# gisbi-kim/lt-mapper

Measured on AMD Instinct MI355X. Metric: keyframe-pairs/sec (removert+diff), higher is better.
Workload: dtype f32; 1 GPU; lot-2x500-os1-64-3res; sensor=os1-64

## Files before the change

include/ltm.h:

```cpp
#ifndef LTM_H
#define LTM_H

#include <stddef.h>
#include <stdint.h>

#ifdef __cplusplus
extern "C" {
#endif

#define LTM_ABI_VERSION 1

enum {
    LTM_OK = 0,
    LTM_E_INVALID = -1,
    LTM_E_DEVICE = -2,
    LTM_E_NOMEM = -3,
    LTM_E_UNSUPPORTED = -4
};

typedef struct ltm_ctx ltm_ctx;
typedef uint64_t ltm_cloud;
typedef uint64_t ltm_scanset;
typedef uint64_t ltm_poses;

// ... 166 lines not shown
int ltm_debug_range_image(ltm_ctx*, ltm_cloud pts, const double* T1, const double* T2, float res_alpha,
                          float* rimg, int32_t* ptidx);
int ltm_debug_viz_images(ltm_ctx*, ltm_cloud map, ltm_scanset scans, ltm_poses poses, size_t kf, float res_alpha, int mode,
                         float range_min, float range_max, float diff_min, float diff_max,
                         uint8_t* scan_bgr, uint8_t* map_bgr, uint8_t* diff_bgr, uint8_t* ptidx_bgr);
int ltm_debug_project(ltm_ctx*, const float* xyz, size_t n, float res_alpha, float* out_az_el_r, int32_t* out_row_col);
void ltm_rimg_size(float vfov, float hfov, float res_alpha, int* rows, int* cols);
int ltm_debug_selfcheck(ltm_ctx*, uint64_t* mismatches3, int* fast_math_enabled);
int ltm_debug_elevation_fit(float vfov_deg, float* c4, double* max_err_rad);
int ltm_debug_pcl_sort_order(const uint32_t* leaf_idx, size_t n, uint32_t* order_out, int use_std_sort, uint32_t* heap_sort_fallbacks );
int ltm_debug_voxel_key_bits(const float* mn3, const float* mx3, float leaf, uint64_t* kept_mask, unsigned* depth, double* frame_min3);
int ltm_debug_cull_check(ltm_ctx*, const float* xyz, size_t n, const double* inv_pose16_or_null, float res_alpha, uint64_t* violations);
int ltm_debug_cull_validation(ltm_ctx*, uint64_t* shapes_checked, uint64_t* shapes_failed);
int ltm_debug_occlusion_stats(ltm_ctx*, uint64_t* pairs, uint64_t* first_shell, uint64_t* projected, int reset);
int ltm_debug_voxel_stats(ltm_ctx*, uint64_t* grids, uint64_t* identity_hits, int reset);
int ltm_debug_knn_stats(ltm_ctx*, uint64_t* queries, uint64_t* undecided, uint64_t* two_phase_calls, uint64_t* unsorted_queue_calls, int reset);
int ltm_debug_sc_paths(int num_ring, int num_sector, int* scatter_in_lds, int* pair_in_lds);
int ltm_debug_cull_stats(ltm_ctx*, uint64_t* survivors, uint64_t* points, int reset);
int ltm_debug_pool_live(ltm_ctx*, uint64_t* live_blocks, uint64_t* live_bytes);

int ltm_profile_enable(ltm_ctx*, int on);
int ltm_profile_reset(ltm_ctx*);
int ltm_profile_read(ltm_ctx*, const char** names, double* ms, uint64_t* launches, double* units, double* bytes, int cap);
int ltm_profile_read_compulsory(ltm_ctx*, double* bytes_c, int cap);

#ifdef __cplusplus
}
#endif
#endif
```

lt-mapper_amd/capi.py:

```python
import ctypes as C
import os

import numpy as np

_HERE = os.path.dirname(os.path.abspath(__file__))
LIB_PATH = os.path.join(_HERE, "libltm_hip.so")

_lib = None

LTM_OK = 0
ERR_NAMES = {0: "LTM_OK", -1: "LTM_E_INVALID", -2: "LTM_E_DEVICE", -3: "LTM_E_NOMEM", -4: "LTM_E_UNSUPPORTED"}


class LtmError(RuntimeError):
    def __init__(self, code, msg):
        super().__init__(f"{ERR_NAMES.get(code, code)}: {msg}")
        self.code = code


class LtmConfig(C.Structure):
    _fields_ = [("vfov", C.c_float), ("hfov", C.c_float), ("lidar2base", C.c_double * 16),
                ("device", C.c_int), ("max_kf_batch", C.c_int)]


# ... 116 lines not shown
    "ltm_submaps_assemble": (_i, [_vp, _u64, _vp, _vp, _sz, _i, _f, _i, _pu64]),
    "ltm_search_build_scanset": (_i, [_vp, _u64, _sz, _sz, C.POINTER(_vp)]),
    "ltm_debug_pool_live": (_i, [_vp, _pu64, _pu64]),
    "ltm_debug_range_image": (_i, [_vp, _u64, _vp, _vp, _f, _vp, _vp]),
    "ltm_debug_viz_images": (_i, [_vp, _u64, _u64, _u64, _sz, _f, _i, _f, _f, _f, _f, _vp, _vp, _vp, _vp]),
    "ltm_debug_project": (_i, [_vp, _vp, _sz, _f, _vp, _vp]),
    "ltm_debug_elevation_fit": (_i, [_f, C.POINTER(_f), C.POINTER(C.c_double)]),
    "ltm_debug_pcl_sort_order": (_i, [C.POINTER(C.c_uint32), C.c_size_t, C.POINTER(C.c_uint32), _i, C.POINTER(C.c_uint32)]),
    "ltm_debug_voxel_key_bits": (_i, [C.POINTER(_f), C.POINTER(_f), _f, _pu64, C.POINTER(C.c_uint), C.POINTER(C.c_double)]),
    "ltm_debug_selfcheck": (_i, [_vp, _pu64, C.POINTER(_i)]),
    "ltm_debug_cull_check": (_i, [_vp, _vp, _sz, _vp, _f, _pu64]),
    "ltm_debug_cull_stats": (_i, [_vp, _pu64, _pu64, _i]),
    "ltm_debug_cull_validation": (_i, [_vp, _pu64, _pu64]),
    "ltm_debug_occlusion_stats": (_i, [_vp, _pu64, _pu64, _pu64, _i]),
    "ltm_debug_voxel_stats": (_i, [_vp, _pu64, _pu64, _i]),
    "ltm_debug_knn_stats": (_i, [_vp, _pu64, _pu64, _pu64, _pu64, _i]),
    "ltm_debug_sc_paths": (_i, [_i, _i, C.POINTER(_i), C.POINTER(_i)]),
    "ltm_rimg_size": (None, [_f, _f, _f, C.POINTER(_i), C.POINTER(_i)]),
    "ltm_profile_enable": (_i, [_vp, _i]),
    "ltm_profile_reset": (_i, [_vp]),
    "ltm_profile_read_compulsory": (_i, [_vp, C.POINTER(C.c_double), _i]),
    "ltm_profile_read": (_i, [_vp, C.POINTER(C.c_char_p), C.POINTER(C.c_double), _pu64, C.POINTER(C.c_double),
                              C.POINTER(C.c_double), _i]),
}


def load_library(path=None):
    global _lib
    if _lib is not None and path is None:
        return _lib
# ... 460 lines not shown
        t = None if inv_pose is None else _mat16(inv_pose)
        v = _u64()
        self._ck(self.lib.ltm_debug_cull_check(self.h, a.ctypes.data, a.shape[0], None if t is None else t.ctypes.data, alpha, C.byref(v)))
        return int(v.value)

    def occlusion_stats(self, reset=False):
        a, b, d = _u64(), _u64(), _u64()
        self._ck(self.lib.ltm_debug_occlusion_stats(self.h, C.byref(a), C.byref(b), C.byref(d), 1 if reset else 0))
        return a.value, b.value, d.value

    def voxel_stats(self, reset=False):
        a, b = _u64(), _u64()
        self._ck(self.lib.ltm_debug_voxel_stats(self.h, C.byref(a), C.byref(b), 1 if reset else 0))
        return int(a.value), int(b.value)

    def knn_stats(self, reset=False):
        q, u, t, s = _u64(), _u64(), _u64(), _u64()
        self._ck(self.lib.ltm_debug_knn_stats(self.h, C.byref(q), C.byref(u), C.byref(t), C.byref(s), 1 if reset else 0))
        return int(q.value), int(u.value), int(t.value), int(s.value)

    def cull_validation(self):
        a, b = _u64(), _u64()
        self._ck(self.lib.ltm_debug_cull_validation(self.h, C.byref(a), C.byref(b)))
        return int(a.value), int(b.value)

    def cull_stats(self, reset=True):
        a, b = _u64(), _u64()
        self._ck(self.lib.ltm_debug_cull_stats(self.h, C.byref(a), C.byref(b), 1 if reset else 0))
        return int(a.value), int(b.value)

# ... 332 lines not shown
```

lt-mapper_amd/csrc/ltm_api_core.cpp:

```cpp
#include "ltm_internal.h"

namespace ltm_detail {

bool inverse4x4(const double* m, double* inv)
{
    double A[2][2], B[2][2], C[2][2], D[2][2];
    for (int r = 0; r < 2; ++r)
        for (int k = 0; k < 2; ++k) {
            A[r][k] = m[4 * k + r]; B[r][k] = m[4 * (k + 2) + r];
            C[r][k] = m[4 * k + r + 2]; D[r][k] = m[4 * (k + 2) + r + 2];
        }
    const double dA = A[0][0] * A[1][1] - A[0][1] * A[1][0], dB = B[0][0] * B[1][1] - B[0][1] * B[1][0];
    const double dC = C[0][0] * C[1][1] - C[0][1] * C[1][0], dD = D[0][0] * D[1][1] - D[0][1] * D[1][0];
    double AB[2][2], DC[2][2];
    for (int j = 0; j < 2; ++j) {
        AB[0][j] = B[0][j] * A[1][1] - B[1][j] * A[0][1]; AB[1][j] = B[1][j] * A[0][0] - B[0][j] * A[1][0];
        DC[0][j] = C[0][j] * D[1][1] - C[1][j] * D[0][1]; DC[1][j] = C[1][j] * D[0][0] - C[0][j] * D[1][0];
    }
    const double tr = (AB[0][0] * DC[0][0] + AB[1][0] * DC[0][1]) + (AB[0][1] * DC[1][0] + AB[1][1] * DC[1][1]);
    double iA[2][2], iB[2][2], iC[2][2], iD[2][2];
    for (int i = 0; i < 2; ++i)
        for (int j = 0; j < 2; ++j) {
            iD[i][j] = D[i][j] * dA - (AB[0][j] * C[i][0] + AB[1][j] * C[i][1]);
            iA[i][j] = A[i][j] * dD - (DC[0][j] * B[i][0] + DC[1][j] * B[i][1]);
// ... 193 lines not shown
    c->kopts.tile_cull = env_int("LTM_TILE_CULL", 1);
    c->kopts.stats_blockmin = env_int("LTM_STATS_BLOCKMIN", 0);
    {
        unsigned long long* d = nullptr;
        bool ok = hipMalloc(&d, 3 * sizeof(unsigned long long)) == hipSuccess && hipMemsetAsync(d, 0, 24, c->stream) == hipSuccess &&
                  selfcheck_fast_math(cfg->vfov, cfg->hfov, d, c->stream) == hipSuccess &&
                  hipMemcpyAsync(c->selfcheck, d, 24, hipMemcpyDeviceToHost, c->stream) == hipSuccess &&
                  hipStreamSynchronize(c->stream) == hipSuccess;
        if (d) (void)hipFree(d);
        if (!ok) { (void)hipStreamDestroy(c->stream); delete c; return LTM_E_DEVICE; }
        c->fast_math = (c->selfcheck[0] == 0 && c->selfcheck[1] == 0 && c->selfcheck[2] == 0) ? 1 : 0;
        if (const char* v = getenv("LTM_KNN_FAST")) c->knn_two_phase = atoi(v);
        if (const char* v = getenv("LTM_VOXEL_KEYBITS")) c->voxel_key_compress = atoi(v);
        if (const char* v = getenv("LTM_VOXEL_FUSED_TAIL")) c->voxel_fused_tail = atoi(v);
        if (const char* v = getenv("LTM_VOXEL_IDENTITY")) c->voxel_identity = atoi(v);
        if (const char* v = getenv("LTM_OCCLUSION")) c->occlusion_cull = atoi(v);
        if (getenv("LTM_OCCLUSION_STATS")) c->occlusion_stats_on = 1;
        if (const char* v = getenv("LTM_OCCLUSION_MIN_PAIRS")) c->occlusion_min_pairs = (size_t)atoll(v);
        if (const char* v = getenv("LTM_OCCLUSION_RNEAR")) {
            const float r = (float)atof(v);
            c->occlusion_r_near = std::isfinite(r) ? std::max(1.0f, r) : 60.0f;
        }
        if (const char* v = getenv("LTM_KNN_STATS")) c->knn_stats_on = atoi(v);
        if (const char* v = getenv("LTM_CULL_SELFCHECK")) c->cull_selfcheck = atoi(v);
        if (const char* v = getenv("LTM_CULL_EPS_SCALE")) c->cull_eps_scale = (float)atof(v);
        if (const char* v = getenv("LTM_CULL_EPS_FLOOR")) c->cull_eps_floor = (float)atof(v);
        c->el_fit = elevation_fit_for(c->cfg.vfov, c->el_c, &c->el_fit_err);
        if (const char* v = getenv("LTM_HEAVY_CHAIN")) c->heavy_chain_on = atoi(v);
        if (const char* v = getenv("LTM_HEAVY_MIN_BLOCKS")) c->heavy_min_blocks = (size_t)atoll(v);
    }
// ... 95 lines not shown
}

int ltm_cloud_device_ptr(ltm_ctx* c, ltm_cloud h, const void** p)
{
    return guarded(c, [&] { LTM_REQUIRE(p, "null argument"); *p = get_cloud(c, h).d; });
}

int ltm_cloud_clone(ltm_ctx* c, ltm_cloud h, ltm_cloud* out)
{
    return guarded(c, [&] {
        LTM_REQUIRE(out, "null argument");
        const Cloud src = get_cloud(c, h);
        float4* d;
        const ltm_cloud nh = alloc_cloud(c, src.n, &d);
        d2d(c, d, src.d, src.n * 16);
        inherit_frame(c, nh, src);
        *out = nh;
    });
}

int ltm_cloud_concat(ltm_ctx* c, const ltm_cloud* in, size_t n, ltm_cloud* out)
{
    return guarded(c, [&] {
        LTM_REQUIRE(out && (in || n == 0), "null argument");
        size_t tot = 0;
        for (size_t i = 0; i < n; ++i) tot += get_cloud(c, in[i]).n;
        float4* d;
        const ltm_cloud h = alloc_cloud(c, tot, &d);
        size_t at = 0;
        for (size_t i = 0; i < n; ++i) { const Cloud& s = get_cloud(c, in[i]); d2d(c, d + at, s.d, s.n * 16); at += s.n; }
        *out = h;
    });
}

int ltm_cloud_transform(ltm_ctx* c, ltm_cloud hin, const double* T1, const double* T2, ltm_cloud* out)
{
    return guarded(c, [&] {
        LTM_REQUIRE(out, "null argument");
        const Cloud in = get_cloud(c, hin);
        float4* d;
        const ltm_cloud h = alloc_cloud(c, in.n, &d);
        HostMat34 a, b;
        if (T1) a = to34(T1);
        if (T2) b = to34(T2);
        if (!T1 && !T2) d2d(c, d, in.d, in.n * 16);
// ... 572 lines not shown
{
    if (!parent || !out) return LTM_E_INVALID;
    *out = nullptr;
    ltm_ctx* c = new (std::nothrow) ltm_ctx();
    if (!c) return LTM_E_NOMEM;
    {
        std::lock_guard<std::recursive_mutex> lk(parent->mx);
        c->cfg = parent->cfg; c->device = parent->device; c->L2B = parent->L2B; c->B2L = parent->B2L;
        c->l2b_identity = parent->l2b_identity; c->b2l_identity = parent->b2l_identity; c->kf_batch = parent->kf_batch; c->kopts = parent->kopts;
        c->fast_math = parent->fast_math;
        for (int i = 0; i < 3; ++i) c->selfcheck[i] = parent->selfcheck[i];
        c->scan_cache_cap = parent->scan_cache_cap; c->occlusion_cull = parent->occlusion_cull;
        c->occlusion_min_pairs = parent->occlusion_min_pairs; c->occlusion_r_near = parent->occlusion_r_near;
        c->occlusion_subtile = parent->occlusion_subtile; c->occlusion_stats_on = parent->occlusion_stats_on;
        c->voxel_key_compress = parent->voxel_key_compress; c->voxel_fused_tail = parent->voxel_fused_tail; c->voxel_identity = parent->voxel_identity;
        c->knn_two_phase = parent->knn_two_phase; c->knn_stats_on = parent->knn_stats_on;
        c->cull_eps_scale = parent->cull_eps_scale; c->cull_eps_floor = parent->cull_eps_floor;
        c->cull_selfcheck = parent->cull_selfcheck; c->cull_geom_ok = parent->cull_geom_ok;
        c->el_fit = parent->el_fit; for (int i = 0; i < 4; ++i) c->el_c[i] = parent->el_c[i]; c->el_fit_err = parent->el_fit_err;
    }
    if (hipSetDevice(c->device) != hipSuccess || hipStreamCreateWithFlags(&c->stream, hipStreamNonBlocking) != hipSuccess) {
        delete c;
        return LTM_E_DEVICE;
    }
    c->pool.stream = c->stream;
    {
        std::lock_guard<std::recursive_mutex> lk(parent->mx);
        c->heavy = parent->heavy;
        c->heavy_chain_on = parent->heavy_chain_on; c->heavy_min_blocks = parent->heavy_min_blocks;
        c->in_lane_family = parent->in_lane_family = true;
// ... 32 lines not shown
    if (!ev) return;
    if (ev->e) { (void)hipSetDevice(ev->device); (void)hipEventDestroy(ev->e); }
    delete ev;
}

static int cloud_pass(ltm_ctx* from, ltm_cloud h, ltm_ctx* to, ltm_cloud* out, bool give)
{
    return guarded2(from, to, [&] {
        LTM_REQUIRE(out, "null argument");
        LTM_REQUIRE(from != to, "lend / give need two contexts");
        const Cloud src = get_cloud(from, h);
        LTM_REQUIRE(!give || !src.borrowed, "a borrowed cloud cannot be given away");
        stream_after(from, to);
        const ltm_cloud nh = new_cloud(to, src.d, src.n);
        Cloud& dst = to->clouds[nh];
        dst.vf_ok = src.vf_ok; dst.vf = src.vf; dst.vleaf = src.vleaf;
        if (give) {
            if (!from->pool.move_to(src.d, to->pool)) { to->clouds.erase(nh); throw Err{LTM_E_INVALID, "cloud memory is not owned by this context's pool"}; }
            from->clouds.erase(h);
        } else dst.borrowed = true;
        *out = nh;
    });
}

int ltm_cloud_lend(ltm_ctx* from, ltm_cloud h, ltm_ctx* to, ltm_cloud* out) { return cloud_pass(from, h, to, out, false); }

int ltm_cloud_give(ltm_ctx* from, ltm_cloud h, ltm_ctx* to, ltm_cloud* out) { return cloud_pass(from, h, to, out, true); }

static int scanset_pass(ltm_ctx* from, ltm_scanset h, ltm_ctx* to, ltm_scanset* out, bool give)
{
    return guarded2(from, to, [&] {
// ... 87 lines not shown
```

lt-mapper_amd/csrc/ltm_api_voxel.cpp:

```cpp
#include "ltm_internal.h"

namespace ltm_detail {

bool octree_frame_from_bbox(const float mn[3], const float mx[3], float leaf, OctreeFrame* f)
{
    const float eps512 = FLT_EPSILON * 512.0f;
    const float minValue = FLT_EPSILON;
    double lo[3], hi[3];
    for (int d = 0; d < 3; ++d) { lo[d] = (double)mn[d]; hi[d] = (double)(float)(mx[d] + eps512); }
    const double res = (double)leaf;
    unsigned mk = 2;
    for (int d = 0; d < 3; ++d) mk = std::max(mk, (unsigned)std::ceil((hi[d] - lo[d] - minValue) / res));
    const unsigned depth = std::min(32u, (unsigned)std::ceil(std::log2((double)mk) - minValue));
    if (depth > 21) return false;
    const double side = (double)(1u << depth) * res;
    for (int d = 0; d < 3; ++d) {
        const double over = (side - (hi[d] - lo[d])) / 2.0;
        if (over > minValue) lo[d] -= over;
    }
    f->minx = lo[0]; f->miny = lo[1]; f->minz = lo[2]; f->res = res; f->depth = depth;
    return true;
}

KeyCompress key_compress_for(const float mn[3], const float mx[3], const OctreeFrame& f, bool enable)
// ... 45 lines not shown
void voxel_segments(ltm_ctx* c, const uint64_t* keys2, size_t n, unsigned kshift, uint32_t* starts, uint32_t* count_dev)
{
    if (c->voxel_fused_tail) {
        const size_t tb = voxel_heads_starts_temp_bytes(n);
        DevBuf temp(c, tb);
        LTM_HIP(voxel_heads_starts(keys2, n, kshift, starts, temp.p, count_dev, c->stream));
        return;
    }
    DevBuf heads(c, n), pos(c, n * 4);
    LTM_HIP(head_flags(keys2, n, heads.as<uint8_t>(), c->stream, kshift));
    scan_flags(c, heads.as<uint8_t>(), n, pos);
    LTM_HIP(scan_total_to(heads.as<uint8_t>(), pos.as<uint32_t>(), n, count_dev, c->stream));
    LTM_HIP(segment_starts(heads.as<uint8_t>(), pos.as<uint32_t>(), n, starts, c->stream));
}

size_t voxel_centroid_raw(ltm_ctx* c, const float4* pts, size_t n_in, float leaf, float4** out, uint32_t shard = 0, uint32_t n_shards = 1,
                          const OctreeFrame* cached = nullptr, OctreeFrame* frame_out = nullptr, const float* box_mn = nullptr, const float* box_mx = nullptr)
{
    *out = nullptr;
    if (n_in == 0) return 0;
    LTM_REQUIRE(leaf > 0.0f, "leaf size must be positive");
    LTM_REQUIRE(n_in < 0xffffffffull, "cloud too large for 32-bit point indices");
    ProfScope p(c, "voxel", (double)n_in, 64.0 * n_in);
    ++c->voxel_calls;
    float mn[3], mx[3];
    bool untouched = false;
    if (cached && c->voxel_identity && n_shards == 1) {
        untouched = read_box(c, mn, mx, [&](uint32_t* bb) { return bbox_reduce_check(pts, n_in, *cached, bb, c->stream); }) == 0;
    } else if (box_mn && box_mx) {
        for (int d = 0; d < 3; ++d) { mn[d] = box_mn[d]; mx[d] = box_mx[d]; }
    } else bbox_of(c, pts, n_in, mn, mx);
    OctreeFrame f;
    if (!octree_frame_from_bbox(mn, mx, leaf, &f)) throw Err{LTM_E_UNSUPPORTED, "octree depth > 21 (extent / leaf too large)"};
    if (frame_out) *frame_out = f;
    if (untouched && same_frame(f, *cached)) {
        float4* o = reinterpret_cast<float4*>(c->pool.alloc(n_in * sizeof(float4)));
        d2d(c, o, pts, n_in * sizeof(float4));
        ++c->voxel_identity_hits;
        *out = o;
        return n_in;
    }
    unsigned ib = 1;
    while (ib < 32 && ((size_t)1 << ib) < n_in) ++ib;
    const KeyCompress kc = key_compress_for(mn, mx, f, c->voxel_key_compress != 0);
    const bool packed = kc.bits + ib <= 64;
    const unsigned mbits = packed ? kc.bits : 3 * f.depth;
    const unsigned kshift = packed ? ib : 0;
    size_t n = n_in;
    DevBuf keys(c, n * 8), idx(c, packed ? 8 : n * 4);
    if (packed) LTM_HIP(morton_keys_packed(pts, n, f, kc, ib, keys.as<uint64_t>(), c->stream));
    else LTM_HIP(morton_keys(pts, n, f, keys.as<uint64_t>(), idx.as<uint32_t>(), c->stream));
    if (n_shards > 1) {
        const unsigned shift = mbits > 12 ? mbits - 12 : 0;
        std::vector<uint32_t> hist(kVoxelKeyBins);
        {
            DevBuf hd(c, kVoxelKeyBins * sizeof(uint32_t));
            LTM_HIP(key_histogram(keys.as<uint64_t>(), n, shift + kshift, hd.as<uint32_t>(), c->stream));
            d2h(c, hist.data(), hd.p, kVoxelKeyBins * sizeof(uint32_t));
        }
        auto cut = [&](uint32_t b) -> uint64_t {
            if (b == 0) return 0;
            if (b >= n_shards) return kVoxelKeyBins;
// ... 8 lines not shown
        auto bound = [&](uint64_t bin) { return bin >= (uint64_t)kVoxelKeyBins ? ~0ull : bin << (shift + kshift); };
        const uint64_t lo = bound(cut(shard));
        const uint64_t hi = (shard + 1 >= n_shards) ? ~0ull : bound(cut(shard + 1));
        DevBuf flags(c, n), pos(c, n * 4);
        LTM_HIP(key_range_flags(keys.as<uint64_t>(), n, lo, hi, flags.as<uint8_t>(), c->stream));
        const size_t nsel = count_flags(c, flags.as<uint8_t>(), n, pos);
        if (nsel == 0) return 0;
        DevBuf ck(c, nsel * 8), ci(c, packed ? 8 : nsel * 4);
        if (packed) LTM_HIP(compact_keys(keys.as<uint64_t>(), flags.as<uint8_t>(), pos.as<uint32_t>(), n, ck.as<uint64_t>(), c->stream));
        else LTM_HIP(compact_pairs(keys.as<uint64_t>(), idx.as<uint32_t>(), flags.as<uint8_t>(), pos.as<uint32_t>(), n,
                                   ck.as<uint64_t>(), ci.as<uint32_t>(), c->stream));
        std::swap(keys.p, ck.p); std::swap(idx.p, ci.p);
        n = nsel;
    }
    DevBuf keys2(c, n * 8), idx2(c, packed ? 8 : n * 4);
    if (packed) {
        const size_t stb = sort_keys_temp_bytes(n);
        DevBuf stemp(c, stb);
        LTM_HIP(sort_keys_u64(keys.as<uint64_t>(), keys2.as<uint64_t>(), n, ib, ib + mbits, stemp.p, stb, c->stream));
    } else {
        const size_t stb = sort_temp_bytes(n);
        DevBuf stemp(c, stb);
        LTM_HIP(sort_pairs_u64(keys.as<uint64_t>(), keys2.as<uint64_t>(), idx.as<uint32_t>(), idx2.as<uint32_t>(), n, mbits, stemp.p, stb, c->stream));
    }
    DevBuf starts(c, n * 4), cnt(c, 4);
    voxel_segments(c, keys2.as<uint64_t>(), n, kshift, starts.as<uint32_t>(), cnt.as<uint32_t>());
    uint32_t nvox32 = 0;
    d2h(c, &nvox32, cnt.p, 4);
    const size_t nvox = nvox32;
    float4* o = reinterpret_cast<float4*>(c->pool.alloc(nvox * sizeof(float4)));
    if (packed) LTM_HIP(voxel_centroids_packed(pts, keys2.as<uint64_t>(), ((uint64_t)1 << ib) - 1, starts.as<uint32_t>(), nvox, n, o, c->stream));
    else LTM_HIP(voxel_centroids(pts, idx2.as<uint32_t>(), starts.as<uint32_t>(), nvox, n, o, c->stream));
    *out = o;
    return nvox;
}

struct VoxelJob {
    const float4* pts; size_t n; float leaf;
    OctreeFrame f; unsigned ib = 1, kshift = 0, mbits = 0; bool packed = false;
    std::unique_ptr<DevBuf> keys, idx, keys2, idx2, starts;
    float4* out = nullptr; size_t nvox = 0;
    bool has_cached = false; OctreeFrame cached{};
    bool identity = false;
};
void voxel_centroid_batch_impl(ltm_ctx* c, std::vector<VoxelJob>& jobs);
void voxel_centroid_batch(ltm_ctx* c, std::vector<VoxelJob>& jobs)
{
    try { voxel_centroid_batch_impl(c, jobs); }
    catch (...) {
        for (VoxelJob& j : jobs) { if (j.out) c->pool.free(j.out); j.out = nullptr; j.nvox = 0; }
        throw;
    }
}
void voxel_centroid_batch_impl(ltm_ctx* c, std::vector<VoxelJob>& jobs)
{
    const size_t nj = jobs.size();
    if (nj == 0) return;
    double tot_pts = 0;
    for (VoxelJob& j : jobs) {
        LTM_REQUIRE(j.leaf > 0.0f || j.n == 0, "leaf size must be positive");
        LTM_REQUIRE(j.n < 0xffffffffull, "cloud too large for 32-bit point indices");
        tot_pts += (double)j.n;
    }
    ProfScope p(c, "voxel", tot_pts, 64.0 * tot_pts);
    DevBuf bb(c, nj * 8 * sizeof(uint32_t));
    for (size_t k = 0; k < nj; ++k) {
        LTM_HIP(bbox_init(bb.as<uint32_t>() + 8 * k, c->stream));
        if (jobs[k].has_cached && c->voxel_identity) LTM_HIP(bbox_reduce_check(jobs[k].pts, jobs[k].n, jobs[k].cached, bb.as<uint32_t>() + 8 * k, c->stream));
        else LTM_HIP(bbox_reduce(jobs[k].pts, jobs[k].n, bb.as<uint32_t>() + 8 * k, c->stream));
    }
    std::vector<uint32_t> enc(nj * 8);
    d2h(c, enc.data(), bb.p, enc.size() * 4);
    DevBuf counts(c, nj * 4);
    for (size_t k = 0; k < nj; ++k) {
        VoxelJob& j = jobs[k];
        if (j.n == 0) { LTM_HIP(hipMemsetAsync(counts.as<uint32_t>() + k, 0, 4, c->stream)); continue; }
        ++c->voxel_calls;
        float mn[3], mx[3];
        decode_box(&enc[8 * k], mn, mx);
        if (!octree_frame_from_bbox(mn, mx, j.leaf, &j.f)) throw Err{LTM_E_UNSUPPORTED, "octree depth > 21 (extent / leaf too large)"};
        if (j.has_cached && c->voxel_identity && enc[8 * k + 6] == 0 && same_frame(j.f, j.cached)) {
            j.identity = true;
            j.out = reinterpret_cast<float4*>(c->pool.alloc(j.n * sizeof(float4)));
            d2d(c, j.out, j.pts, j.n * sizeof(float4));
            LTM_HIP(fill_u32(counts.as<uint32_t>() + k, (uint32_t)j.n, 1, c->stream));
            ++c->voxel_identity_hits;
            continue;
        }
        while (j.ib < 32 && ((size_t)1 << j.ib) < j.n) ++j.ib;
        const KeyCompress kc = key_compress_for(mn, mx, j.f, c->voxel_key_compress != 0);
        j.packed = kc.bits + j.ib <= 64;
        j.mbits = j.packed ? kc.bits : 3 * j.f.depth;
        j.kshift = j.packed ? j.ib : 0;
        const size_t n = j.n;
        j.keys.reset(new DevBuf(c, n * 8)); j.idx.reset(new DevBuf(c, j.packed ? 8 : n * 4));
        j.keys2.reset(new DevBuf(c, n * 8)); j.idx2.reset(new DevBuf(c, j.packed ? 8 : n * 4));
        if (j.packed) {
            LTM_HIP(morton_keys_packed(j.pts, n, j.f, kc, j.ib, j.keys->as<uint64_t>(), c->stream));
            const size_t stb = sort_keys_temp_bytes(n);
            DevBuf stemp(c, stb);
            LTM_HIP(sort_keys_u64(j.keys->as<uint64_t>(), j.keys2->as<uint64_t>(), n, j.ib, j.ib + j.mbits, stemp.p, stb, c->stream));
        } else {
            LTM_HIP(morton_keys(j.pts, n, j.f, j.keys->as<uint64_t>(), j.idx->as<uint32_t>(), c->stream));
            const size_t stb = sort_temp_bytes(n);
            DevBuf stemp(c, stb);
            LTM_HIP(sort_pairs_u64(j.keys->as<uint64_t>(), j.keys2->as<uint64_t>(), j.idx->as<uint32_t>(), j.idx2->as<uint32_t>(), n, j.mbits, stemp.p, stb, c->stream));
        }
        j.keys.reset(); j.idx.reset();
        j.starts.reset(new DevBuf(c, n * 4));
        voxel_segments(c, j.keys2->as<uint64_t>(), n, j.kshift, j.starts->as<uint32_t>(), counts.as<uint32_t>() + k);
    }
    std::vector<uint32_t> nv(nj);
    d2h(c, nv.data(), counts.p, nj * 4);
    for (size_t k = 0; k < nj; ++k) {
        VoxelJob& j = jobs[k];
        j.nvox = nv[k];
// ... 6 lines not shown
}


}

extern "C" {

int ltm_voxel_centroid(ltm_ctx* c, ltm_cloud hin, float leaf, ltm_cloud* out)
{
    return guarded(c, [&] {
        LTM_REQUIRE(out, "null argument");
        const Cloud in = get_cloud(c, hin);
        float4* d = nullptr;
        OctreeFrame f{};
        const bool have = in.vf_ok && in.vleaf == leaf;
        const size_t nv = voxel_centroid_raw(c, in.d, in.n, leaf, &d, 0, 1, have ? &in.vf : nullptr, &f);
        if (!d) d = reinterpret_cast<float4*>(c->pool.alloc(sizeof(float4)));
        *out = new_cloud(c, d, nv);
        if (in.n) set_frame(c, *out, f, leaf, true);
    });
}

int ltm_voxel_centroid_batch(ltm_ctx* c, size_t n, const ltm_cloud* in, const float* leaf, ltm_cloud* out)
{
    return guarded(c, [&] {
        LTM_REQUIRE((in && leaf && out) || n == 0, "null argument");
        std::vector<VoxelJob> jobs(n);
        for (size_t k = 0; k < n; ++k) {
            const Cloud cl = get_cloud(c, in[k]);
            jobs[k].pts = cl.d; jobs[k].n = cl.n; jobs[k].leaf = leaf[k];
            jobs[k].has_cached = cl.vf_ok && cl.vleaf == leaf[k] && cl.n > 0;
            jobs[k].cached = cl.vf;
        }
        voxel_centroid_batch(c, jobs);
        size_t done = 0;
        try {
            for (; done < n; ++done) {
                float4* d = jobs[done].out ? jobs[done].out : reinterpret_cast<float4*>(c->pool.alloc(sizeof(float4)));
                jobs[done].out = nullptr;
                out[done] = new_cloud(c, d, jobs[done].nvox);
                if (jobs[done].n) set_frame(c, out[done], jobs[done].f, jobs[done].leaf, true);
            }
        } catch (...) {
            for (size_t k = done; k < n; ++k) if (jobs[k].out) c->pool.free(jobs[k].out);
            throw;
        }
    });
// ... 383 lines not shown
    if (!octree_frame_from_bbox(mn3, mx3, leaf, &f)) return LTM_E_UNSUPPORTED;
    const KeyCompress kc = key_compress_for(mn3, mx3, f, true);
    uint64_t m = 0;
    for (int r = 0; r < kc.n_runs; ++r) m |= kc.mask[r] << kc.src[r];
    *kept_mask = m;
    if (depth) *depth = f.depth;
    if (frame_min3) { frame_min3[0] = f.minx; frame_min3[1] = f.miny; frame_min3[2] = f.minz; }
    return (int)kc.bits;
}

int ltm_debug_voxel_stats(ltm_ctx* c, uint64_t* grids, uint64_t* identity_hits, int reset)
{
    return guarded(c, [&] {
        if (grids) *grids = c->voxel_calls;
        if (identity_hits) *identity_hits = c->voxel_identity_hits;
        if (reset) c->voxel_calls = c->voxel_identity_hits = 0;
    });
}

}

int ltm_detail::voxel_grid_scanset_ordered(ltm_ctx* c, ltm_scanset hin, float leaf, int order, ltm_scanset* out)
{
    ltm_vgs* t = nullptr;
    const int rc = guarded(c, [&] { vgs_begin(c, hin, leaf, order, &t); });
    if (rc != LTM_OK) return rc;
    return ltm_voxel_grid_scanset_end(c, t, out);
}

void ltm_detail::vgs_release_all(ltm_ctx* c)
{
// ... 6 lines not shown
```

lt-mapper_amd/csrc/ltm_internal.h:

```cpp
#pragma once
#include "ltm.h"
#include "ltm_pclsort.h"
#include "ltm_kernels.h"
#include "ltm_device_prims.h"

#include <hip/hip_runtime_api.h>

#include <algorithm>
#include <atomic>
#include <chrono>
#include <condition_variable>
#include <deque>
#include <mutex>
#include <thread>
#include <cfloat>
#include <climits>
#include <cmath>
#include <cstdio>
#include <cstdlib>
#include <cstring>
#include <map>
#include <memory>
#include <new>
#include <string>
// ... 129 lines not shown
    void release_all()
    {
        for (auto& kv : foreign) send_home(kv.first, kv.second, false);
        foreign.clear();
        { std::lock_guard<std::mutex> lk(inbox->mx); inbox->closed = true; }
        release_cached();
        for (auto& kv : live) (void)hipFree(kv.first);
        live.clear();
    }
};

struct Cloud {
    float4* d = nullptr; size_t n = 0;
    bool borrowed = false;
    bool vf_ok = false; OctreeFrame vf{}; float vleaf = 0.0f;
};
struct ScanSet { float4* d = nullptr; size_t n_pts = 0; std::vector<uint64_t> off; uint64_t* off_dev = nullptr; bool borrowed = false; size_t nkf() const { return off.size() - 1; } };
struct Poses { size_t n = 0; std::vector<double> pose, inv; double* pose_dev = nullptr; double* inv_dev = nullptr; float* approx_dev = nullptr; };

struct ProfClass { double ms = 0; uint64_t launches = 0; double units = 0, bytes = 0, bytes_c = 0; };
struct ScanImgEntry { uint64_t ss; int rows, cols; size_t kb, nb; uint32_t* buf; uint32_t* smax; size_t bytes; uint64_t stamp; float* qbound; float q_thr; };
struct Pending { int cls; hipEvent_t a, b; };
struct PendingLive { int cls; int slot; double max_pts; double image_bytes; double map_pts; double image_bytes_c; };
struct PinnedBlock { void* p; size_t bytes; bool in_use; };
struct UploadState { float4* d = nullptr; size_t cap = 0, n = 0; std::vector<uint64_t> off{0}; void* stage[2] = {nullptr, nullptr}; size_t stage_sz[2] = {0, 0}; hipEvent_t ev[2] = {nullptr, nullptr}; bool busy[2] = {false, false}; int next = 0; size_t fill = 0, flushed = 0; };

}
using namespace ltm_detail;

struct FetchChunk { void* host; size_t first_point, n_points, first_kf, n_kf; };
// ... 65 lines not shown
    std::vector<ScanImgEntry> scan_cache;
    uint64_t scan_cache_stamp = 0;
    size_t scan_cache_cap = (size_t)3 << 30;
    int occlusion_cull = 1;
    size_t occlusion_min_pairs = (size_t)1 << 21;
    float occlusion_r_near = 60.0f;
    int occlusion_subtile = 1;
    int occlusion_stats_on = 0;
    uint64_t occl_quarters = 0, occl_quarters_live = 0;
    uint64_t occl_pairs = 0, occl_near = 0, occl_far_live = 0;
    void* occl_scratch = nullptr; size_t occl_scratch_bytes = 0;
    int voxel_key_compress = 1;
    int voxel_fused_tail = 1;
    int voxel_identity = 1;
    uint64_t voxel_identity_hits = 0, voxel_calls = 0;
    int knn_two_phase = 1;
    int knn_stats_on = 0;
    uint64_t knn_undecided = 0, knn_queries = 0;
    uint64_t knn_two_phase_calls = 0, knn_unsorted_calls = 0;
    std::map<std::pair<int, int>, bool> cull_geom_ok;
    uint64_t cull_geoms_checked = 0, cull_geoms_failed = 0;
    int cull_selfcheck = 1;
    float cull_eps_scale = 0.0f;
    float cull_eps_floor = 1.0e-3f;
    int el_fit = 0;
    float el_c[4] = {1.0f, 0.0f, 0.0f, 0.0f};
    double el_fit_err = 0.0;
    void* scratch_pinned = nullptr;
    hipStream_t copy_stream = nullptr;
    std::vector<PinnedBlock> pinned;
// ... 163 lines not shown
{
    const uint64_t h = c->next_handle++;
    Cloud cl; cl.d = d; cl.n = n;
    c->clouds[h] = cl;
    return h;
}
inline void inherit_frame(ltm_ctx* c, ltm_cloud child, const Cloud& parent)
{
    if (!parent.vf_ok) return;
    Cloud& ch = c->clouds[child];
    ch.vf_ok = true; ch.vf = parent.vf; ch.vleaf = parent.vleaf;
}
inline void set_frame(ltm_ctx* c, ltm_cloud h, const OctreeFrame& f, float leaf, bool ok)
{
    Cloud& cl = c->clouds[h];
    cl.vf_ok = ok; cl.vf = f; cl.vleaf = leaf;
}
inline ltm_cloud alloc_cloud(ltm_ctx* c, size_t n, float4** d)
{
    *d = reinterpret_cast<float4*>(c->pool.alloc(std::max<size_t>(n, 1) * sizeof(float4)));
    return new_cloud(c, *d, n);
}
inline ltm_scanset new_scanset(ltm_ctx* c, float4* d, std::vector<uint64_t> off)
{
    ScanSet s;
    s.d = d; s.n_pts = off.back(); s.off = std::move(off);
    s.off_dev = reinterpret_cast<uint64_t*>(c->pool.alloc(s.off.size() * sizeof(uint64_t)));
    h2d(c, s.off_dev, s.off.data(), s.off.size() * sizeof(uint64_t));
    const uint64_t h = c->next_handle++;
    c->scansets[h] = std::move(s);
    return h;
// ... 140 lines not shown
```

lt-mapper_amd/csrc/ltm_k_voxel.hip:

```cpp
#include "ltm_kernels_common.h"
#include <rocprim/device/device_radix_sort.hpp>
#include <rocprim/device/device_scan.hpp>
namespace ltm {

__global__ void k_bbox_init(uint32_t* b)
{
    if (threadIdx.x < 3) b[threadIdx.x] = 0xffffffffu;
    else if (threadIdx.x < 8) b[threadIdx.x] = 0u;
}
hipError_t bbox_init(uint32_t* bbox, hipStream_t s)
{
    k_bbox_init<<<dim3(1), dim3(64), 0, s>>>(bbox);
    return hipGetLastError();
}
__global__ void __launch_bounds__(kBlock)
k_bbox_reduce(const float4* __restrict__ pts, size_t n, uint32_t* __restrict__ bbox)
{
    BoxAcc box;
    const size_t stride = (size_t)gridDim.x * blockDim.x;
    size_t i = (size_t)blockIdx.x * blockDim.x + threadIdx.x;
    for (; i + 3 * stride < n; i += 4 * stride) {
        float4 p[4];
#pragma unroll
        for (int u = 0; u < 4; ++u) p[u] = pts[i + (size_t)u * stride];
// ... 190 lines not shown
{
    size_t bytes = 0;
    uint64_t* k = nullptr;
    (void)rocprim::radix_sort_keys(nullptr, bytes, k, k, n ? n : 1, 0, 64);
    return bytes + 256;
}
hipError_t sort_keys_u64(const uint64_t* keys_in, uint64_t* keys_out, size_t n, unsigned begin_bit, unsigned end_bit, void* temp,
                         size_t temp_bytes, hipStream_t s)
{
    if (!n) return hipSuccess;
    if (end_bit > 64) end_bit = 64;
    if (end_bit <= begin_bit) end_bit = begin_bit + 1;
    return rocprim::radix_sort_keys(temp, temp_bytes, keys_in, keys_out, n, begin_bit, end_bit, s);
}

size_t sort_temp_bytes(size_t n)
{
    size_t bytes = 0;
    uint64_t* k = nullptr; uint32_t* v = nullptr;
    (void)rocprim::radix_sort_pairs(nullptr, bytes, k, k, v, v, n ? n : 1, 0, 64);
    return bytes + 256;
}
hipError_t sort_pairs_u64(const uint64_t* keys_in, uint64_t* keys_out, const uint32_t* val_in, uint32_t* val_out, size_t n,
                          unsigned end_bit, void* temp, size_t temp_bytes, hipStream_t s)
{
    if (!n) return hipSuccess;
    if (end_bit < 1) end_bit = 1;
    if (end_bit > 64) end_bit = 64;
    return rocprim::radix_sort_pairs(temp, temp_bytes, keys_in, keys_out, val_in, val_out, n, 0, end_bit, s);
}
// ... 214 lines not shown
```

lt-mapper_amd/csrc/ltm_kernels.h:

```cpp
#pragma once
#include <hip/hip_runtime_api.h>
#include <stddef.h>
#include <stdint.h>

namespace ltm {

struct Geom {
    float vfov, hfov;
    int rows, cols;
    int fast;
    float cull_eps_px;
    int el_fit;
    float el_c[4];
    float el_tclamp;
};

struct HostMat34 { double m[12]; };

static const uint32_t kNoPointBits = 0x461C4000u;

hipError_t fill_u32(uint32_t* p, uint32_t v, size_t n, hipStream_t s);
hipError_t fill_u64(uint64_t* p, uint64_t v, size_t n, hipStream_t s);

hipError_t scan_range_images(const float4* scans, const uint64_t* offsets_dev, size_t kb, size_t nb,
// ... 75 lines not shown
hipError_t voxelgrid_keys_seg(const float4* pts, const uint64_t* offsets_dev, size_t n_kf, uint64_t n, const VoxelGridFrame* frames_dev,
                              uint64_t* keys, uint32_t* idx, hipStream_t s);
hipError_t voxelgrid_centroids(const float4* pts, const uint64_t* sorted_keys, const uint32_t* sorted_idx, const uint32_t* starts,
                               const VoxelGridFrame* frames_dev, size_t n_vox, size_t n, float4* out, hipStream_t s);
size_t sort_temp_bytes(size_t n);
hipError_t scan_total_to(const uint8_t* flags, const uint32_t* pos, size_t n, uint32_t* out_dev, hipStream_t s);
hipError_t sort_pairs_u64(const uint64_t* keys_in, uint64_t* keys_out, const uint32_t* val_in, uint32_t* val_out, size_t n,
                          unsigned end_bit, void* temp, size_t temp_bytes, hipStream_t s);
hipError_t head_flags(const uint64_t* keys, size_t n, uint8_t* heads, hipStream_t s, unsigned shift = 0);
static constexpr int kMaxKeyRuns = 24;
struct KeyCompress { int n_runs; unsigned bits; unsigned char src[kMaxKeyRuns], dst[kMaxKeyRuns]; uint64_t mask[kMaxKeyRuns]; };
hipError_t morton_keys_packed(const float4* pts, size_t n, OctreeFrame f, KeyCompress kc, unsigned idx_bits, uint64_t* keys, hipStream_t s);
size_t sort_keys_temp_bytes(size_t n);
hipError_t sort_keys_u64(const uint64_t* keys_in, uint64_t* keys_out, size_t n, unsigned begin_bit, unsigned end_bit, void* temp,
                         size_t temp_bytes, hipStream_t s);
hipError_t voxel_centroids_packed(const float4* pts, const uint64_t* sorted_keys, uint64_t idx_mask, const uint32_t* starts, size_t n_vox,
                                  size_t n, float4* out, hipStream_t s);
hipError_t compact_keys(const uint64_t* keys, const uint8_t* flags, const uint32_t* pos, size_t n, uint64_t* keys_out, hipStream_t s);
static constexpr int kVoxelKeyBins = 4096;
hipError_t key_histogram(const uint64_t* keys, size_t n, unsigned shift, uint32_t* hist, hipStream_t s);
hipError_t key_range_flags(const uint64_t* keys, size_t n, uint64_t lo, uint64_t hi, uint8_t* flags, hipStream_t s);
hipError_t compact_pairs(const uint64_t* keys, const uint32_t* idx, const uint8_t* flags, const uint32_t* pos, size_t n,
                         uint64_t* keys_out, uint32_t* idx_out, hipStream_t s);
hipError_t segment_starts(const uint8_t* heads, const uint32_t* pos, size_t n, uint32_t* starts, hipStream_t s);
hipError_t voxel_centroids(const float4* pts, const uint32_t* sorted_idx, const uint32_t* starts, size_t n_vox, size_t n,
                           float4* out, hipStream_t s);

struct KnnGrid { double ox, oy, oz, inv_cell; long long nx, ny, nz; };
hipError_t cell_keys(const float4* pts, size_t n, KnnGrid g, uint64_t* keys, uint32_t* idx, hipStream_t s);
hipError_t gather_points(const float4* in, const uint32_t* idx, size_t n, float4* out, hipStream_t s);
// ... 91 lines not shown
```

Before: 3207 keyframe-pairs/s.

## Merge pre-sorted voxelized head with radix-sorted tail when downsampling concatenated clouds

Concatenated clouds now remember how many leading points came from an already-voxelized cloud, along with its octree frame and leaf. When such a cloud is voxel-downsampled again with the same leaf and frame, only the new tail is radix-sorted, and it is then merged with the head's already-sorted packed keys using rocprim::merge. The goal is to avoid re-sorting the large head on every incremental map update. This adds provenance bookkeeping, an extra temporary buffer and merge pass, and a fallback when the bbox check shows the frame has changed.

```diff
diff --git a/include/ltm.h b/include/ltm.h
--- a/include/ltm.h
+++ b/include/ltm.h
@@ -204,6 +204,7 @@
 int ltm_debug_cull_validation(ltm_ctx*, uint64_t* shapes_checked, uint64_t* shapes_failed);
 int ltm_debug_occlusion_stats(ltm_ctx*, uint64_t* pairs, uint64_t* first_shell, uint64_t* projected, int reset);
 int ltm_debug_voxel_stats(ltm_ctx*, uint64_t* grids, uint64_t* identity_hits, int reset);
+int ltm_debug_voxel_merge_stats(ltm_ctx*, uint64_t* merged_grids, uint64_t* head_points, uint64_t* tail_points, int reset);
 int ltm_debug_knn_stats(ltm_ctx*, uint64_t* queries, uint64_t* undecided, uint64_t* two_phase_calls, uint64_t* unsorted_queue_calls, int reset);
 int ltm_debug_sc_paths(int num_ring, int num_sector, int* scatter_in_lds, int* pair_in_lds);
 int ltm_debug_cull_stats(ltm_ctx*, uint64_t* survivors, uint64_t* points, int reset);
diff --git a/lt-mapper_amd/capi.py b/lt-mapper_amd/capi.py
--- a/lt-mapper_amd/capi.py
+++ b/lt-mapper_amd/capi.py
@@ -154,6 +154,7 @@
     "ltm_debug_cull_validation": (_i, [_vp, _pu64, _pu64]),
     "ltm_debug_occlusion_stats": (_i, [_vp, _pu64, _pu64, _pu64, _i]),
     "ltm_debug_voxel_stats": (_i, [_vp, _pu64, _pu64, _i]),
+    "ltm_debug_voxel_merge_stats": (_i, [_vp, _pu64, _pu64, _pu64, _i]),
     "ltm_debug_knn_stats": (_i, [_vp, _pu64, _pu64, _pu64, _pu64, _i]),
     "ltm_debug_sc_paths": (_i, [_i, _i, C.POINTER(_i), C.POINTER(_i)]),
     "ltm_rimg_size": (None, [_f, _f, _f, C.POINTER(_i), C.POINTER(_i)]),
@@ -644,6 +645,11 @@
         self._ck(self.lib.ltm_debug_voxel_stats(self.h, C.byref(a), C.byref(b), 1 if reset else 0))
         return int(a.value), int(b.value)
 
+    def voxel_merge_stats(self, reset=False):
+        a, b, d = _u64(), _u64(), _u64()
+        self._ck(self.lib.ltm_debug_voxel_merge_stats(self.h, C.byref(a), C.byref(b), C.byref(d), 1 if reset else 0))
+        return int(a.value), int(b.value), int(d.value)
+
     def knn_stats(self, reset=False):
         q, u, t, s = _u64(), _u64(), _u64(), _u64()
         self._ck(self.lib.ltm_debug_knn_stats(self.h, C.byref(q), C.byref(u), C.byref(t), C.byref(s), 1 if reset else 0))
diff --git a/lt-mapper_amd/csrc/ltm_api_core.cpp b/lt-mapper_amd/csrc/ltm_api_core.cpp
--- a/lt-mapper_amd/csrc/ltm_api_core.cpp
+++ b/lt-mapper_amd/csrc/ltm_api_core.cpp
@@ -231,6 +231,7 @@
         if (const char* v = getenv("LTM_VOXEL_KEYBITS")) c->voxel_key_compress = atoi(v);
         if (const char* v = getenv("LTM_VOXEL_FUSED_TAIL")) c->voxel_fused_tail = atoi(v);
         if (const char* v = getenv("LTM_VOXEL_IDENTITY")) c->voxel_identity = atoi(v);
+        if (const char* v = getenv("LTM_VOXEL_MERGE")) c->voxel_merge = atoi(v);
         if (const char* v = getenv("LTM_OCCLUSION")) c->occlusion_cull = atoi(v);
         if (getenv("LTM_OCCLUSION_STATS")) c->occlusion_stats_on = 1;
         if (const char* v = getenv("LTM_OCCLUSION_MIN_PAIRS")) c->occlusion_min_pairs = (size_t)atoll(v);
@@ -356,7 +357,7 @@
         float4* d;
         const ltm_cloud nh = alloc_cloud(c, src.n, &d);
         d2d(c, d, src.d, src.n * 16);
-        inherit_frame(c, nh, src);
+        copy_provenance(c->clouds[nh], src);
         *out = nh;
     });
 }
@@ -371,6 +372,11 @@
         const ltm_cloud h = alloc_cloud(c, tot, &d);
         size_t at = 0;
         for (size_t i = 0; i < n; ++i) { const Cloud& s = get_cloud(c, in[i]); d2d(c, d + at, s.d, s.n * 16); at += s.n; }
+        if (n) {
+            const Cloud first = get_cloud(c, in[0]);
+            const size_t head = first.vf_ok ? first.n : first.vhead;
+            if (head) { Cloud& o = c->clouds[h]; o.vf = first.vf; o.vleaf = first.vleaf; o.vhead = head; }
+        }
         *out = h;
     });
 }
@@ -973,6 +979,7 @@
         c->occlusion_min_pairs = parent->occlusion_min_pairs; c->occlusion_r_near = parent->occlusion_r_near;
         c->occlusion_subtile = parent->occlusion_subtile; c->occlusion_stats_on = parent->occlusion_stats_on;
         c->voxel_key_compress = parent->voxel_key_compress; c->voxel_fused_tail = parent->voxel_fused_tail; c->voxel_identity = parent->voxel_identity;
+        c->voxel_merge = parent->voxel_merge;
         c->knn_two_phase = parent->knn_two_phase; c->knn_stats_on = parent->knn_stats_on;
         c->cull_eps_scale = parent->cull_eps_scale; c->cull_eps_floor = parent->cull_eps_floor;
         c->cull_selfcheck = parent->cull_selfcheck; c->cull_geom_ok = parent->cull_geom_ok;
@@ -1035,7 +1042,7 @@
         stream_after(from, to);
         const ltm_cloud nh = new_cloud(to, src.d, src.n);
         Cloud& dst = to->clouds[nh];
-        dst.vf_ok = src.vf_ok; dst.vf = src.vf; dst.vleaf = src.vleaf;
+        copy_provenance(dst, src);
         if (give) {
             if (!from->pool.move_to(src.d, to->pool)) { to->clouds.erase(nh); throw Err{LTM_E_INVALID, "cloud memory is not owned by this context's pool"}; }
             from->clouds.erase(h);
diff --git a/lt-mapper_amd/csrc/ltm_api_voxel.cpp b/lt-mapper_amd/csrc/ltm_api_voxel.cpp
--- a/lt-mapper_amd/csrc/ltm_api_voxel.cpp
+++ b/lt-mapper_amd/csrc/ltm_api_voxel.cpp
@@ -83,8 +83,36 @@
     LTM_HIP(segment_starts(heads.as<uint8_t>(), pos.as<uint32_t>(), n, starts, c->stream));
 }
 
+hipError_t bbox_head_tail(const float4* pts, size_t n, size_t n_head, const OctreeFrame& head_frame, uint32_t* bbox8, hipStream_t s)
+{
+    const hipError_t e = bbox_reduce_check(pts, n_head, head_frame, bbox8, s);
+    return e != hipSuccess ? e : bbox_reduce(pts + n_head, n - n_head, bbox8, s);
+}
+static constexpr size_t kMergeMinHeadPerTail = 4;
+size_t merge_head_of(const ltm_ctx* c, const Cloud& cl, float leaf)
+{
+    if (!c->voxel_merge || cl.vf_ok || cl.vhead == 0 || cl.vhead >= cl.n || cl.vleaf != leaf) return 0;
+    return (cl.n - cl.vhead) * kMergeMinHeadPerTail <= cl.vhead ? cl.vhead : 0;
+}
+void voxel_sort_packed(ltm_ctx* c, const uint64_t* keys, uint64_t* keys2, size_t n, size_t n_head, unsigned ib, unsigned mbits)
+{
+    const size_t n_sort = n - n_head;
+    const size_t stb = sort_keys_temp_bytes(n_sort);
+    if (n_head == 0) {
+        DevBuf stemp(c, stb);
+        LTM_HIP(sort_keys_u64(keys, keys2, n, ib, ib + mbits, stemp.p, stb, c->stream));
+        return;
+    }
+    const size_t mtb = merge_keys_temp_bytes(n_head, n_sort);
+    DevBuf tail(c, n_sort * 8), temp(c, std::max(stb, mtb));
+    LTM_HIP(sort_keys_u64(keys + n_head, tail.as<uint64_t>(), n_sort, ib, ib + mbits, temp.p, stb, c->stream));
+    LTM_HIP(merge_keys_u64(keys, n_head, tail.as<uint64_t>(), n_sort, keys2, temp.p, mtb, c->stream));
+    ++c->voxel_merge_hits; c->voxel_merge_head_pts += n_head; c->voxel_merge_tail_pts += n_sort;
+}
+
 size_t voxel_centroid_raw(ltm_ctx* c, const float4* pts, size_t n_in, float leaf, float4** out, uint32_t shard = 0, uint32_t n_shards = 1,
-                          const OctreeFrame* cached = nullptr, OctreeFrame* frame_out = nullptr, const float* box_mn = nullptr, const float* box_mx = nullptr)
+                          const OctreeFrame* cached = nullptr, OctreeFrame* frame_out = nullptr, const float* box_mn = nullptr, const float* box_mx = nullptr,
+                          size_t n_head = 0)
 {
     *out = nullptr;
     if (n_in == 0) return 0;
@@ -93,8 +121,10 @@
     ProfScope p(c, "voxel", (double)n_in, 64.0 * n_in);
     ++c->voxel_calls;
     float mn[3], mx[3];
-    bool untouched = false;
-    if (cached && c->voxel_identity && n_shards == 1) {
+    bool untouched = false, head_sorted = false;
+    if (cached && n_head) {
+        head_sorted = read_box(c, mn, mx, [&](uint32_t* bb) { return bbox_head_tail(pts, n_in, n_head, *cached, bb, c->stream); }) == 0;
+    } else if (cached && c->voxel_identity && n_shards == 1) {
         untouched = read_box(c, mn, mx, [&](uint32_t* bb) { return bbox_reduce_check(pts, n_in, *cached, bb, c->stream); }) == 0;
     } else if (box_mn && box_mx) {
         for (int d = 0; d < 3; ++d) { mn[d] = box_mn[d]; mx[d] = box_mx[d]; }
@@ -115,6 +145,7 @@
     const bool packed = kc.bits + ib <= 64;
     const unsigned mbits = packed ? kc.bits : 3 * f.depth;
     const unsigned kshift = packed ? ib : 0;
+    const size_t n_merge = (head_sorted && packed && same_frame(f, *cached)) ? n_head : 0;
     size_t n = n_in;
     DevBuf keys(c, n * 8), idx(c, packed ? 8 : n * 4);
     if (packed) LTM_HIP(morton_keys_packed(pts, n, f, kc, ib, keys.as<uint64_t>(), c->stream));
@@ -153,11 +184,8 @@
         n = nsel;
     }
     DevBuf keys2(c, n * 8), idx2(c, packed ? 8 : n * 4);
-    if (packed) {
-        const size_t stb = sort_keys_temp_bytes(n);
-        DevBuf stemp(c, stb);
-        LTM_HIP(sort_keys_u64(keys.as<uint64_t>(), keys2.as<uint64_t>(), n, ib, ib + mbits, stemp.p, stb, c->stream));
-    } else {
+    if (packed) voxel_sort_packed(c, keys.as<uint64_t>(), keys2.as<uint64_t>(), n, n_merge, ib, mbits);
+    else {
         const size_t stb = sort_temp_bytes(n);
         DevBuf stemp(c, stb);
         LTM_HIP(sort_pairs_u64(keys.as<uint64_t>(), keys2.as<uint64_t>(), idx.as<uint32_t>(), idx2.as<uint32_t>(), n, mbits, stemp.p, stb, c->stream));
@@ -180,6 +208,7 @@
     std::unique_ptr<DevBuf> keys, idx, keys2, idx2, starts;
     float4* out = nullptr; size_t nvox = 0;
     bool has_cached = false; OctreeFrame cached{};
+    size_t n_head = 0;
     bool identity = false;
 };
 void voxel_centroid_batch_impl(ltm_ctx* c, std::vector<VoxelJob>& jobs);
@@ -205,7 +234,8 @@
     DevBuf bb(c, nj * 8 * sizeof(uint32_t));
     for (size_t k = 0; k < nj; ++k) {
         LTM_HIP(bbox_init(bb.as<uint32_t>() + 8 * k, c->stream));
-        if (jobs[k].has_cached && c->voxel_identity) LTM_HIP(bbox_reduce_check(jobs[k].pts, jobs[k].n, jobs[k].cached, bb.as<uint32_t>() + 8 * k, c->stream));
+        if (jobs[k].n_head) LTM_HIP(bbox_head_tail(jobs[k].pts, jobs[k].n, jobs[k].n_head, jobs[k].cached, bb.as<uint32_t>() + 8 * k, c->stream));
+        else if (jobs[k].has_cached && c->voxel_identity) LTM_HIP(bbox_reduce_check(jobs[k].pts, jobs[k].n, jobs[k].cached, bb.as<uint32_t>() + 8 * k, c->stream));
         else LTM_HIP(bbox_reduce(jobs[k].pts, jobs[k].n, bb.as<uint32_t>() + 8 * k, c->stream));
     }
     std::vector<uint32_t> enc(nj * 8);
@@ -235,10 +265,9 @@
         j.keys.reset(new DevBuf(c, n * 8)); j.idx.reset(new DevBuf(c, j.packed ? 8 : n * 4));
         j.keys2.reset(new DevBuf(c, n * 8)); j.idx2.reset(new DevBuf(c, j.packed ? 8 : n * 4));
         if (j.packed) {
+            const bool merge = j.n_head && enc[8 * k + 6] == 0 && same_frame(j.f, j.cached);
             LTM_HIP(morton_keys_packed(j.pts, n, j.f, kc, j.ib, j.keys->as<uint64_t>(), c->stream));
-            const size_t stb = sort_keys_temp_bytes(n);
-            DevBuf stemp(c, stb);
-            LTM_HIP(sort_keys_u64(j.keys->as<uint64_t>(), j.keys2->as<uint64_t>(), n, j.ib, j.ib + j.mbits, stemp.p, stb, c->stream));
+            voxel_sort_packed(c, j.keys->as<uint64_t>(), j.keys2->as<uint64_t>(), n, merge ? j.n_head : 0, j.ib, j.mbits);
         } else {
             LTM_HIP(morton_keys(j.pts, n, j.f, j.keys->as<uint64_t>(), j.idx->as<uint32_t>(), c->stream));
             const size_t stb = sort_temp_bytes(n);
@@ -275,7 +304,8 @@
         float4* d = nullptr;
         OctreeFrame f{};
         const bool have = in.vf_ok && in.vleaf == leaf;
-        const size_t nv = voxel_centroid_raw(c, in.d, in.n, leaf, &d, 0, 1, have ? &in.vf : nullptr, &f);
+        const size_t n_head = merge_head_of(c, in, leaf);
+        const size_t nv = voxel_centroid_raw(c, in.d, in.n, leaf, &d, 0, 1, (have || n_head) ? &in.vf : nullptr, &f, nullptr, nullptr, n_head);
         if (!d) d = reinterpret_cast<float4*>(c->pool.alloc(sizeof(float4)));
         *out = new_cloud(c, d, nv);
         if (in.n) set_frame(c, *out, f, leaf, true);
@@ -292,6 +322,7 @@
             jobs[k].pts = cl.d; jobs[k].n = cl.n; jobs[k].leaf = leaf[k];
             jobs[k].has_cached = cl.vf_ok && cl.vleaf == leaf[k] && cl.n > 0;
             jobs[k].cached = cl.vf;
+            jobs[k].n_head = merge_head_of(c, cl, leaf[k]);
         }
         voxel_centroid_batch(c, jobs);
         size_t done = 0;
@@ -705,7 +736,17 @@
     return guarded(c, [&] {
         if (grids) *grids = c->voxel_calls;
         if (identity_hits) *identity_hits = c->voxel_identity_hits;
-        if (reset) c->voxel_calls = c->voxel_identity_hits = 0;
+        if (reset) c->voxel_calls = c->voxel_identity_hits = c->voxel_merge_hits = c->voxel_merge_head_pts = c->voxel_merge_tail_pts = 0;
+    });
+}
+
+int ltm_debug_voxel_merge_stats(ltm_ctx* c, uint64_t* merged_grids, uint64_t* head_points, uint64_t* tail_points, int reset)
+{
+    return guarded(c, [&] {
+        if (merged_grids) *merged_grids = c->voxel_merge_hits;
+        if (head_points) *head_points = c->voxel_merge_head_pts;
+        if (tail_points) *tail_points = c->voxel_merge_tail_pts;
+        if (reset) c->voxel_merge_hits = c->voxel_merge_head_pts = c->voxel_merge_tail_pts = 0;
     });
 }
 
diff --git a/lt-mapper_amd/csrc/ltm_internal.h b/lt-mapper_amd/csrc/ltm_internal.h
--- a/lt-mapper_amd/csrc/ltm_internal.h
+++ b/lt-mapper_amd/csrc/ltm_internal.h
@@ -167,6 +167,7 @@
     float4* d = nullptr; size_t n = 0;
     bool borrowed = false;
     bool vf_ok = false; OctreeFrame vf{}; float vleaf = 0.0f;
+    size_t vhead = 0;
 };
 struct ScanSet { float4* d = nullptr; size_t n_pts = 0; std::vector<uint64_t> off; uint64_t* off_dev = nullptr; bool borrowed = false; size_t nkf() const { return off.size() - 1; } };
 struct Poses { size_t n = 0; std::vector<double> pose, inv; double* pose_dev = nullptr; double* inv_dev = nullptr; float* approx_dev = nullptr; };
@@ -262,6 +263,8 @@
     int voxel_fused_tail = 1;
     int voxel_identity = 1;
     uint64_t voxel_identity_hits = 0, voxel_calls = 0;
+    int voxel_merge = 1;
+    uint64_t voxel_merge_hits = 0, voxel_merge_head_pts = 0, voxel_merge_tail_pts = 0;
     int knn_two_phase = 1;
     int knn_stats_on = 0;
     uint64_t knn_undecided = 0, knn_queries = 0;
@@ -455,7 +458,11 @@
 inline void set_frame(ltm_ctx* c, ltm_cloud h, const OctreeFrame& f, float leaf, bool ok)
 {
     Cloud& cl = c->clouds[h];
-    cl.vf_ok = ok; cl.vf = f; cl.vleaf = leaf;
+    cl.vf_ok = ok; cl.vf = f; cl.vleaf = leaf; cl.vhead = 0;
+}
+inline void copy_provenance(Cloud& dst, const Cloud& src)
+{
+    dst.vf_ok = src.vf_ok; dst.vf = src.vf; dst.vleaf = src.vleaf; dst.vhead = src.vhead;
 }
 inline ltm_cloud alloc_cloud(ltm_ctx* c, size_t n, float4** d)
 {
diff --git a/lt-mapper_amd/csrc/ltm_k_voxel.hip b/lt-mapper_amd/csrc/ltm_k_voxel.hip
--- a/lt-mapper_amd/csrc/ltm_k_voxel.hip
+++ b/lt-mapper_amd/csrc/ltm_k_voxel.hip
@@ -1,4 +1,5 @@
 #include "ltm_kernels_common.h"
+#include <rocprim/device/device_merge.hpp>
 #include <rocprim/device/device_radix_sort.hpp>
 #include <rocprim/device/device_scan.hpp>
 namespace ltm {
@@ -228,6 +229,19 @@
     return rocprim::radix_sort_keys(temp, temp_bytes, keys_in, keys_out, n, begin_bit, end_bit, s);
 }
 
+size_t merge_keys_temp_bytes(size_t n_a, size_t n_b)
+{
+    size_t bytes = 0;
+    uint64_t* k = nullptr;
+    (void)rocprim::merge(nullptr, bytes, k, k, k, n_a ? n_a : 1, n_b ? n_b : 1);
+    return bytes + 256;
+}
+hipError_t merge_keys_u64(const uint64_t* a, size_t n_a, const uint64_t* b, size_t n_b, uint64_t* out, void* temp, size_t temp_bytes, hipStream_t s)
+{
+    if (!n_a && !n_b) return hipSuccess;
+    return rocprim::merge(temp, temp_bytes, a, b, out, n_a, n_b, rocprim::less<uint64_t>(), s);
+}
+
 size_t sort_temp_bytes(size_t n)
 {
     size_t bytes = 0;
diff --git a/lt-mapper_amd/csrc/ltm_kernels.h b/lt-mapper_amd/csrc/ltm_kernels.h
--- a/lt-mapper_amd/csrc/ltm_kernels.h
+++ b/lt-mapper_amd/csrc/ltm_kernels.h
@@ -113,6 +113,8 @@
 size_t sort_keys_temp_bytes(size_t n);
 hipError_t sort_keys_u64(const uint64_t* keys_in, uint64_t* keys_out, size_t n, unsigned begin_bit, unsigned end_bit, void* temp,
                          size_t temp_bytes, hipStream_t s);
+size_t merge_keys_temp_bytes(size_t n_a, size_t n_b);
+hipError_t merge_keys_u64(const uint64_t* a, size_t n_a, const uint64_t* b, size_t n_b, uint64_t* out, void* temp, size_t temp_bytes, hipStream_t s);
 hipError_t voxel_centroids_packed(const float4* pts, const uint64_t* sorted_keys, uint64_t idx_mask, const uint32_t* starts, size_t n_vox,
                                   size_t n, float4* out, hipStream_t s);
 hipError_t compact_keys(const uint64_t* keys, const uint8_t* flags, const uint32_t* pos, size_t n, uint64_t* keys_out, hipStream_t s);
```

Result: no change. 3203 keyframe-pairs/s (-0.1%).
